# archibate/ptina

Measured on AMD Instinct MI355X. Metric: Msamples/sec (pixels x spp / s), 512x512x32spp cornell-monkey (978 tri), higher is better.
Workload: dtype f32; 1 GPU; s978: 978-tri synthetic cornell + bumpy sphere, 512x512, 32 spp, unidirectional MIS path tracer, depth<=5; step = 32 x render() + get_image() (resolve + D2H), exams/benchmark.py:29-36; spp=32, mode=fast, parallelism=single GPU

## Files before the change

### ptina_amd/csrc/lds_layout.h

```cpp
#pragma once

#if defined(__HIPCC__)
#define MPT_LDS_FN __host__ __device__ static inline
#else
#define MPT_LDS_FN static inline
#endif

#ifndef MPT_LDS_NODE_STRIDE
#define MPT_LDS_NODE_STRIDE 72
#endif
#ifndef MPT_LDS4_NODE_STRIDE
#define MPT_LDS4_NODE_STRIDE 112
#endif
#define MPT_LDS_MAT_VEC4 6

enum {
    MPT_LDS_BUDGET = 160 * 1024,
    MPT_LDS_LANES = 1024,
    MPT_LDS_LEVEL_BYTES = MPT_LDS_LANES * 2
};

typedef struct { int nnode4, ntri4, nmat4, nmtl4; } MptLdsRegions;

MPT_LDS_FN MptLdsRegions mpt_lds_regions(int n, int default_mtl) {
    MptLdsRegions r;
    r.nnode4 = ((n - 1) * MPT_LDS_NODE_STRIDE + 15) >> 4;
    r.ntri4 = n * 3;
    r.nmat4 = (default_mtl + 1) * MPT_LDS_MAT_VEC4;
    r.nmtl4 = (n + 15) >> 4;
    return r;
}

MPT_LDS_FN MptLdsRegions mpt_lds4_regions(int n, int nwide, int lds_nmats) {
    MptLdsRegions r;
    r.nnode4 = nwide * (MPT_LDS4_NODE_STRIDE / 16);
    r.ntri4 = (n + 1) * 3;
    r.nmat4 = (lds_nmats + 1) * MPT_LDS_MAT_VEC4;
    r.nmtl4 = (n + 15) >> 4;
    return r;
}

MPT_LDS_FN int mpt_lds_scene_vec4(MptLdsRegions r) { return r.nnode4 + r.ntri4 + r.nmat4 + r.nmtl4; }

MPT_LDS_FN int mpt_lds_launch_bytes(MptLdsRegions r, int stack_levels) {
    return mpt_lds_scene_vec4(r) * 16 + stack_levels * MPT_LDS_LEVEL_BYTES;
}

MPT_LDS_FN int mpt_lds_stack_levels(int fast_depth) { return fast_depth + 1; }

static inline int mpt_lds_fit_bytes(int n, int max_materials, int fast_depth) {
    if (n < 2) return 0;
    if (n >= 32768) return 0;
    if ((n - 1) * (MPT_LDS_NODE_STRIDE / 8) >= 32768) return 0;
    if (max_materials >= 256) return 0;
    if (fast_depth < 0 || fast_depth >= MPT_LDS_BUDGET / MPT_LDS_LEVEL_BYTES) return 0;
    const int bytes = mpt_lds_launch_bytes(mpt_lds_regions(n, max_materials), mpt_lds_stack_levels(fast_depth));
    return bytes <= MPT_LDS_BUDGET ? bytes : 0;
}

static inline int mpt_lds4_fit_bytes(int n, int nwide, int wide_stack, int lds_nmats) {
    if (n < 2 || nwide <= 0 || wide_stack <= 0) return 0;
    if (n >= 4095) return 0;
    if (nwide > 65535 / MPT_LDS4_NODE_STRIDE) return 0;
    if (lds_nmats < 0 || lds_nmats >= 255) return 0;
    if (wide_stack > MPT_LDS_BUDGET / MPT_LDS_LEVEL_BYTES) return 0;
    const int bytes = mpt_lds_launch_bytes(mpt_lds4_regions(n, nwide, lds_nmats), wide_stack);
    return bytes <= MPT_LDS_BUDGET ? bytes : 0;
}

enum { MPT_KERNEL_GATHER = 0, MPT_KERNEL_LDS = 1, MPT_KERNEL_WIDE = 2, MPT_KERNEL_LDS4 = 5 };

typedef struct {
    int fast;
    int use_lds;
    int lds_wide;
    int use_wide;
    int nfaces;
    int wide_nodes;
    int wide_stack;
    int have_wnode;
    int max_mtlid;
    int max_materials;
    int fast_depth;
} MptKernelFacts;

typedef struct { int kernel, lds_bytes; } MptKernelChoice;

static inline MptKernelChoice mpt_choose_kernel(const MptKernelFacts *f) {
    MptKernelChoice ch = { MPT_KERNEL_GATHER, 0 };
    if (!f->fast) return ch;
    if (f->use_lds) {
        if (f->lds_wide && f->use_wide && f->have_wnode)
            ch.lds_bytes = mpt_lds4_fit_bytes(f->nfaces, f->wide_nodes, f->wide_stack, f->max_mtlid + 1);
        if (ch.lds_bytes) { ch.kernel = MPT_KERNEL_LDS4; return ch; }
        ch.lds_bytes = mpt_lds_fit_bytes(f->nfaces, f->max_materials, f->fast_depth);
        if (ch.lds_bytes) { ch.kernel = MPT_KERNEL_LDS; return ch; }
    }
    if (f->use_wide && f->wide_nodes > 0) ch.kernel = MPT_KERNEL_WIDE;
    return ch;
}
```

### ptina_amd/csrc/miptina.cpp

```cpp

#include "miptina_ctx.h"
#include <chrono>

static int g_hwq = 0;
static bool g_hwq_late = false;
__attribute__((constructor)) static void mpt_want_hw_queues() {
    if (!getenv("GPU_MAX_HW_QUEUES")) {
        setenv("GPU_MAX_HW_QUEUES", "12", 0);
        const char *pre = getenv("LD_PRELOAD");
        if ((pre && strstr(pre, "rocprof")) || getenv("ROCP_TOOL_LIBRARIES")) {
            g_hwq_late = true;
            fprintf(stderr, "libmiptina: GPU_MAX_HW_QUEUES=12 requested after a preloaded profiler tool may have initialised HIP: "
                            "streams may fold onto the default 4 hardware queues (results unchanged; export the variable "
                            "before starting the profiler)\n");
        }
    }
    const char *v = getenv("GPU_MAX_HW_QUEUES");
    g_hwq = v ? atoi(v) : 0;
}

static thread_local std::string g_err;

int fail(const char *fmt, ...) {
    char buf[1024];
// ... 205 lines not shown

static bool is_locked_range(const void *p, size_t bytes) {
    std::lock_guard<std::mutex> lk(g_host_mu);
    auto it = g_host_bufs.upper_bound((uintptr_t)p);
    if (it == g_host_bufs.begin()) return false;
    --it;
    return (uintptr_t)p + bytes <= it->first + it->second;
}

static int read_back(mpt_ctx *c, void *out, const void *dev, size_t bytes) {
    if (is_locked_range(out, bytes)) {
        HIP_TRY(hipMemcpyAsync(out, dev, bytes, hipMemcpyDeviceToHost, c->stream));
        HIP_TRY(hipStreamSynchronize(c->stream));
        return 0;
    }
    if (bytes > c->h_stage_bytes) {
        if (c->h_stage) hipHostFree(c->h_stage);
        c->h_stage = nullptr; c->h_stage_bytes = 0;
        HIP_TRY(hipHostMalloc(&c->h_stage, bytes, hipHostMallocDefault));
        c->h_stage_bytes = bytes;
    }
    HIP_TRY(hipMemcpyAsync(c->h_stage, dev, bytes, hipMemcpyDeviceToHost, c->stream));
    HIP_TRY(hipStreamSynchronize(c->stream));
    memcpy(out, c->h_stage, bytes);
    return 0;
}

static int scene_feat_now(const mpt_ctx *c);

extern "C" int mpt_set_option(mpt_ctx *c, const char *key, int value) {
    if (use(c)) return 1;
    std::string k = key ? key : "";
    if (k == "mode") {
        if (value != MPT_MODE_FAST && value != MPT_MODE_STRICT) return fail("mode must be 0 (fast) or 1 (strict)");
        c->mode = value;
    } else if (k == "batch") {
        if (value < 1 || value > MPT_MAX_BATCH) return fail("batch must be in 1..%d", MPT_MAX_BATCH);
        c->batch = value;
    } else if (k == "chunk") {
        if (value < 0) return fail("chunk must be >= 0");
        c->chunk = value;
    } else if (k == "count") {
        c->count = value ? 1 : 0;
    } else if (k == "lds") {
        c->use_lds = value ? 1 : 0;
    } else if (k == "lds_wide") {
        if (value != 0 && value != 1) return fail("lds_wide must be 0 or 1");
        c->lds_wide = value;
    } else if (k == "zero_copy") {
        c->zero_copy = value ? 1 : 0;
    } else if (k == "shade_spec") {
        if (value != 0 && value != 1) return fail("shade_spec must be 0 (always the generic SHADE) or 1 (the plain one for plain scenes)");
        c->shade_spec = value;
    } else if (k == "skip_dark") {
        if (value < -1 || value > 1) return fail("skip_dark must be -1 (auto), 0 or 1");
        c->skip_dark = value;
    } else if (k == "spin_us") {
        if (value < 0) return fail("spin_us must be >= 0");
        c->spin_us = value;
    } else if (k == "finalise") {
        if (value < 0 || value > 2) return fail("finalise must be 0 (combine pass), 1 (tail finalisation) or 2 (the same without the early image: A/B)");
        c->finalise = value;
    } else if (k == "launch_seq") {
        if (value < 0) return fail("launch_seq must be >= 0");
        if (mpt_flush(c)) return 1;
        c->launch_seq = (unsigned)value;
        c->tag_epoch = 0xffffffffu;
    } else if (k == "timeline") {
        c->timeline = value ? 1 : 0;
    } else if (k == "pipe_depth") {
        if (value != 0 && (value < 2 || value > MPT_MAX_PIPE)) return fail("pipe_depth must be 0 (auto) or 2..%d", MPT_MAX_PIPE);
        c->pipe_depth = value;
    } else if (k == "grid_div") {
        if (value < 0 || value > 8) return fail("grid_div must be 0 (auto) or 1..8");
        c->grid_div = value;
    } else if (k == "lds_block") {
        if (value != 0 && value != 256 && value != 512 && value != 768 && value != 1024)
            return fail("lds_block must be 0 (auto), 256, 512, 768 or 1024");
        c->lds_block = value;
    } else if (k == "reserve_cus") {
        if (value < 0 || value >= c->num_cus) return fail("reserve_cus must be in 0..%d", c->num_cus - 1);
        c->reserve_cus = value;
    } else if (k == "wide") {
        c->use_wide = value ? 1 : 0;
    } else if (k == "sah_exact_max") {
        if (value < 2) return fail("sah_exact_max must be >= 2");
        c->sah_exact_max = value; c->tree_valid = false;
    } else if (k == "sah_build") {
        if (value < -1 || value > 1) return fail("sah_build must be -1 (auto), 0 (host) or 1 (device)");
        if (value != c->sah_build) { c->sah_build = value; c->tree_valid = false; }
    } else if (k == "wide_build") {
        if ((value ? 1 : 0) != c->wide_build) { c->wide_build = value ? 1 : 0; c->tree_valid = false; }
    } else if (k == "wide_quant") {
        c->use_quant = value ? 1 : 0;
    } else if (k == "tree") {
        if (value != 0 && value != 1) return fail("tree must be 0 (LBVH) or 1 (SAH)");
        if (value != c->tree_kind) { c->tree_kind = value; c->tree_valid = false; }
    } else if (k == "tile_w_shift" || k == "tile_h_shift") {
        if (value < 0 || value > 3) return fail("%s must be in 0..3", k.c_str());
        (k == "tile_w_shift" ? c->tile_w_shift : c->tile_h_shift) = value;
    } else if (k == "gpu_build") {
        if ((value ? 1 : 0) != c->gpu_build) { c->gpu_build = value ? 1 : 0; c->tree_valid = false; }
    } else if (k == "sah_inject_fail") {
        c->sah_inject_fail = value != 0; c->tree_valid = false;
    } else if (k == "build_phases") {
        c->build_phases = value ? 1 : 0;
    } else if (k == "lane_hist") {
        c->lane_hist = value ? 1 : 0;
    } else if (k == "sah_max") {
        c->sah_max = value; c->tree_valid = false;
    } else {
        return fail("unknown option '%s'", k.c_str());
    }
    return 0;
}

extern "C" int mpt_get_option(mpt_ctx *c, const char *key, int *value) {
    if (!c || !value) return fail("null argument");
    std::string k = key ? key : "";
    if (k == "mode") *value = c->mode;
    else if (k == "batch") *value = c->batch;
    else if (k == "chunk") *value = c->chunk;
    else if (k == "count") *value = c->count;
    else if (k == "tree_depth") *value = c->tree_depth;
    else if (k == "fast_depth") *value = c->fast_depth;
    else if (k == "tree") *value = c->tree_kind;
    else if (k == "gpu_build") *value = c->gpu_build;
    else if (k == "pending") *value = c->pending;
    else if (k == "lds") *value = c->use_lds;
    else if (k == "lds_wide") *value = c->lds_wide;
    else if (k == "lds_block") *value = c->lds_block;
    else if (k == "zero_copy") *value = c->zero_copy;
    else if (k == "spin_us") *value = c->spin_us;
    else if (k == "finalise") *value = c->finalise;
    else if (k == "last_finalised") *value = c->last_finalised;
    else if (k == "launch_seq") *value = (int)(c->launch_seq & 0x7fffffffu);
    else if (k == "tag_wraps") *value = (int)c->tag_wraps;
    else if (k == "skip_dark") *value = c->skip_dark;
    else if (k == "shade_spec") *value = c->shade_spec;
    else if (k == "scene_feat") *value = scene_feat_now(c);
    else if (k == "shade_inst") *value = c->last_shade_feat;
    else if (k == "pipe_depth") *value = c->pipe_depth;
    else if (k == "grid_div") *value = c->grid_div;
    else if (k == "cur_depth") *value = c->cur_depth;
    else if (k == "cur_div") *value = c->cur_div;
    else if (k == "last_div") *value = c->last_div;
    else if (k == "last_kernel") *value = c->last_kernel;
    else if (k == "num_cus") *value = c->num_cus;
    else if (k == "reserve_cus") *value = c->reserve_cus;
    else if (k == "wide") *value = c->use_wide;
    else if (k == "wide_quant") *value = c->use_quant;
    else if (k == "wide_build") *value = c->wide_build;
    else if (k == "sah_build") *value = c->sah_build;
    else if (k == "sah_fallback") *value = c->sah_fallback;
    else if (k == "build_phases") *value = c->build_phases;
    else if (k == "lane_hist") *value = c->lane_hist;
    else if (k == "sah_levels") *value = c->sah_stats.levels;
    else if (k == "sah_kelems") *value = (int)(c->sah_stats.elems / 1000);
    else if (k == "sah_chunks") *value = (int)c->sah_stats.chunks;
    else if (k == "sah_segments") *value = (int)c->sah_stats.segments;
    else if (k == "sah_part_kwords") *value = (int)(c->sah_stats.part_words / 1000);
    else if (k == "sah_tasks_small") *value = c->sah_stats.tasks_small;
    else if (k == "sah_tasks_big") *value = c->sah_stats.tasks_big;
    else if (k == "sah_t_sort_k") *value = c->sah_stats.t_sort_k;
    else if (k == "sah_t_loop_k") *value = c->sah_stats.t_loop_k;
    else if (k == "sah_t_max_k") *value = c->sah_stats.t_max_k;
    else if (k == "sah_task_levels") *value = c->sah_stats.task_levels;
    else if (k == "sah_task_levels_max") *value = c->sah_stats.task_levels_max;
    else if (k.rfind("build_phase_us_", 0) == 0 && k.size() == 16 && k[15] >= '0' && k[15] <= '5') *value = (int)(c->build_phase_us[k[15] - '0'] + 0.5);
    else if (k == "wide_nodes") *value = c->wide_nodes;
    else if (k == "wide_stack") *value = c->wide_stack;
    else if (k == "wide_ratio_permille") *value = (int)(c->wide_ratio * 1000.f + 0.5f);
    else if (k == "wide_depth") *value = c->wide_depth;
    else if (k == "nranks") *value = c->nranks;
    else if (k == "rank") *value = c->rank;
    else if (k == "device") *value = c->device;
    else if (k == "clock_khz") *value = c->clock_khz;
    else if (k == "hw_queues") *value = g_hwq_late ? -g_hwq : g_hwq;
    else return fail("unknown option '%s'", k.c_str());
    return 0;
}

extern "C" int mpt_set_size(mpt_ctx *c, int nx, int ny) {
    if (use(c)) return 1;
    if (nx <= 0 || ny <= 0) return fail("film size must be positive, got %dx%d", nx, ny);
    size_t npix = (size_t)nx * ny;
    if (npix > (size_t)c->caps.max_filmsize)
        return fail("film %dx%d exceeds max_filmsize=%d (init_things(max_filmsize=...))", nx, ny, c->caps.max_filmsize);
    if (npix > c->film_cap) {
        HIP_TRY(hipStreamSynchronize(c->stream));
        for (int p = 0; p < 3; p++) { hipFree(c->film[p]); c->film[p] = nullptr; }
        hipFree(c->resolved); c->resolved = nullptr;
// ... 519 lines not shown
    switch (kc.kernel) {
    case MPT_KERNEL_LDS4: HIP_TRY(mpt_launch_render_lds4(&p, launch_cus, lds_block, (size_t)kc.lds_bytes, c->count, shade_feat, s.rs)); break;
    case MPT_KERNEL_LDS: HIP_TRY(mpt_launch_render_lds(&p, launch_cus, lds_block, (size_t)kc.lds_bytes, c->count, s.rs)); break;
    case MPT_KERNEL_WIDE: HIP_TRY(mpt_launch_render_wide(&p, wide_blocks, c->count, c->use_quant, s.rs)); break;
    default:
        if (!s.fast) HIP_TRY(mpt_launch_render_strict(&p, p.ntiles, stack, c->count, s.rs));
        else HIP_TRY(mpt_launch_render_fast(&p, launch_cus, stack, c->count, s.rs));
    }
    c->last_shade_feat = shade_feat;
    c->last_kernel = kc.kernel;
    HIP_TRY(hipEventRecord(e1, s.rs));
    c->render_timer.record({ e0, e1 }, c->event_pool);
    return 0;
}

static int behind_launch(mpt_ctx *c, const MptRenderParams &p, const BatchSlot &s, int B, bool fin) {
    const int k = s.k;
    HIP_TRY(hipEventRecord(c->ev_render[k], s.rs));
    HIP_TRY(hipStreamWaitEvent(c->stream, c->ev_render[k], 0));
    if (!fin)
        HIP_TRY(mpt_launch_combine(c->film[0], c->partial2[k], c->ny, c->x0, c->x1, p.stripe_w, p.stripe_pitch,
                                   p.partial_stride / std::max(c->ny, 1), B, c->stream));
    HIP_TRY(hipEventRecord(c->ev_free[k], c->stream));
    const int k2 = c->flip % c->cur_depth;
    if (k2 != k) {
        HIP_TRY(hipStreamWaitEvent(s.ss, c->ev_render[k2], 0));
        HIP_TRY(mpt_launch_sobol_update(c->sX, c->sX_spec, c->sV, c->sP2[k2], c->sdim, c->srows, c->stime, B, B, 1, s.ss));
        HIP_TRY(hipMemsetAsync(c->d_work2[k2], 0, MPT_QUEUE_WORDS * sizeof(unsigned int), s.ss));
        HIP_TRY(hipEventRecord(c->ev_sobol2[k2], s.ss));
        c->spec_valid = true; c->spec_slot = k2; c->spec_B = B; c->spec_time = c->stime;
    }
    return 0;
}

extern "C" int mpt_flush(mpt_ctx *c) {
    if (!c) return fail("null context");
    if (c->mlt_pending && mlt_flush(c)) return 1;
    if (c->pending == 0) return 0;
    HIP_TRY(hipSetDevice(c->device));
    const int B = c->pending;
    c->pending = 0;
    MptRenderParams p;
    if (fill_params(c, p, B)) return 1;
    const bool fast = c->mode == MPT_MODE_FAST;
    if (fast && ring_policy(c, B)) return 1;
    BatchSlot s;
    s.fast = fast;
    s.k = fast ? (c->flip++ % c->cur_depth) : 0;
    s.rs = fast ? c->rstream[s.k] : c->stream;
    s.ss = fast ? c->aux : c->stream;
    bool use_spec = false;
    if (batch_points(c, p, s, B, &use_spec)) return 1;
    if (p.ntiles == 0) return 0;
    const MptKernelChoice kc = choose_kernel(c);
    p.lds_nmats = c->max_mtlid + 1;
    const int ccols = work_items(c, p, B, fast);
    if (fast && slab_and_queue_heads(c, p, s, B, ccols, use_spec)) return 1;
    bool ring_idle = false;
    int launch_cus = 0, wide_blocks = 0, lds_block = 0;
    if (launch_share(c, fast, &ring_idle, &launch_cus)) return 1;
    if (size_launch_buffers(c, p, s.k, kc.kernel, launch_cus, &wide_blocks, &lds_block)) return 1;
    const bool fin = fast && c->finalise && ring_idle && p.nitems > 0;
    if (setup_finalisation(c, p, s, fin)) return 1;
    if (launch_render(c, p, s, kc, launch_cus, lds_block, wide_blocks)) return 1;
    return fast ? behind_launch(c, p, s, B, fin) : 0;
}

extern "C" int mpt_render(mpt_ctx *c, int nframes) {
    if (!c) return fail("null context");
    if (nframes < 0) return fail("nframes must be >= 0");
    if (check_ready(c)) return 1;
    if (c->mlt_pending && mlt_flush(c)) return 1;
    while (nframes > 0) {
        int room = c->batch - c->pending;
        int take = std::min(room, nframes);
        c->pending += take;
        nframes -= take;
        if (c->pending >= c->batch && mpt_flush(c)) return 1;
    }
    return 0;
}

extern "C" int mpt_render_preview(mpt_ctx *c, int nframes) {
    if (use(c)) return 1;
    while (nframes > 0) {
        int B = std::min(nframes, MPT_MAX_BATCH);
        MptRenderParams p;
        if (fill_params(c, p, B)) return 1;
        if (sobol_advance(c, B, B)) return 1;
        p.chunk = B; p.nchunks = 1;
        const int stack = gather_stack_levels(c);
        if (p.ntiles) {
            if (c->mode == MPT_MODE_STRICT) HIP_TRY(mpt_launch_preview_strict(&p, p.ntiles, stack, c->stream));
            else HIP_TRY(mpt_launch_preview_fast(&p, p.ntiles, stack, c->stream));
        }
        nframes -= B;
    }
    return 0;
}

enum { MPT_MLT_SLAB_RECORDS = 1 << 24 };

static int mlt_check(mpt_ctx *c) {
    if (c->mlt_n <= 0) return fail("Metropolis engine not reset: call mpt_mlt_reset first");
    return 0;
}

// ... 440 lines not shown
```

### ptina_amd/csrc/miptina_ctx.h

```cpp
#pragma once

#include "../../include/miptina.h"
#include "mpt_types.h"
#include "shade_feat.h"
#include <hip/hip_runtime_api.h>
#include <rccl/rccl.h>
#include <dlfcn.h>
#include <algorithm>
#include <cmath>
#include <cstdarg>
#include <cstdio>
#include <chrono>
#include <cstring>
#include <initializer_list>
#include <map>
#include <mutex>
#include <string>
#include <vector>

MPT_KERNEL_API hipError_t mpt_launch_render_fast(const MptRenderParams *, int grid, int stack, int count, hipStream_t);
MPT_KERNEL_API hipError_t mpt_launch_render_strict(const MptRenderParams *, int grid, int stack, int count, hipStream_t);
MPT_KERNEL_API hipError_t mpt_launch_derive_materials(MptMaterial *mats, int count, hipStream_t);
MPT_KERNEL_API hipError_t mpt_launch_derive_tfast(const MptVec4 *tgeo, MptVec4 *tfast, int n, hipStream_t);
MPT_KERNEL_API hipError_t mpt_wide_blocks(int grid, int count, int quant, int *blocks);
// ... 53 lines not shown
#define MPT_INTERNAL __attribute__((visibility("hidden")))
MPT_INTERNAL int fail(const char *fmt, ...);

#define HIP_TRY(expr)                                                                     \
    do {                                                                                  \
        hipError_t e_ = (expr);                                                           \
        if (e_ != hipSuccess) return fail("%s failed: %s", #expr, hipGetErrorString(e_)); \
    } while (0)

struct MPT_INTERNAL MptLaunchTimer {
    const int per_launch;
    std::vector<hipEvent_t> events;
    explicit MptLaunchTimer(int n) : per_launch(n) {}

    void record(std::initializer_list<hipEvent_t> launch, std::vector<hipEvent_t> &pool) {
        for (hipEvent_t e : launch) events.push_back(e);
        if (events.size() > (size_t)per_launch * 4096) trim(pool);
    }
    void trim(std::vector<hipEvent_t> &pool) {
        const size_t half = (size_t)per_launch * 2048;
        for (size_t q = 0; q < half; q++) pool.push_back(events[q]);
        events.erase(events.begin(), events.begin() + half);
    }
    int drain(double *seg_ms, int *launches, std::vector<hipEvent_t> &pool) {
        for (size_t q = 0; q + per_launch <= events.size(); q += per_launch)
            for (int g = 0; g + 1 < per_launch; g++) {
                float t = 0;
                HIP_TRY(hipEventElapsedTime(&t, events[q + g], events[q + g + 1]));
                seg_ms[g] += t;
            }
        if (launches) *launches = (int)(events.size() / per_launch);
        for (hipEvent_t e : events) pool.push_back(e);
        events.clear();
        return 0;
    }
};

enum { MPT_MAX_PIPE = 6 };

struct mpt_ctx {
    int device = 0;
    hipStream_t stream = nullptr;
    mpt_caps caps{};

    int mode = MPT_MODE_FAST, batch = 32, chunk = 0, count = 0, use_lds = 1, lds_block = 0, zero_copy = 1;
    int lds_wide = 1;
    int skip_dark = -1;
    int max_mtlid = -1;
    int num_cus = 256;
    int clock_khz = 0;
    int tile_w_shift = 3, tile_h_shift = 3;
    int last_div = 1;
    int last_kernel = 0;
    int shade_spec = 1;
    int last_shade_feat = -1;

    int nx = 0, ny = 0, x0 = 0, x1 = 0;
    int stripe_w = 0, stripe_idx = 0, stripe_mod = 1;
    MptVec4 *film[3] = { nullptr, nullptr, nullptr };
    size_t film_cap = 0;
    MptVec4 *resolved = nullptr;
    float *exported = nullptr;

    int nfaces = 0;
    std::vector<float> verts;
    double scene_cen[3] = { 0, 0, 0 }, scene_rad = 0;
    std::vector<int32_t> mtlids;
    bool tree_valid = false;
    int tree_depth = 0;
    int fast_depth = 0;
    int tree_kind = 1;
    int gpu_build = 1;
    int sah_max = 1 << 22;
    bool host_tree_valid = false;
    float *d_verts = nullptr; int *d_mtlids = nullptr; size_t d_model_cap = 0;
    float *d_cen = nullptr; int *d_bounds = nullptr; int *d_depth = nullptr;
    unsigned long long *d_keys_in = nullptr, *d_keys_out = nullptr;
    void *d_sort_tmp = nullptr; size_t d_sort_bytes = 0;
    int *d_child = nullptr, *d_parent = nullptr, *d_leaf = nullptr, *d_mc = nullptr;
    float *d_bmin = nullptr, *d_bmax = nullptr;
    unsigned *d_arrive = nullptr;
    size_t d_build_cap = 0;
    std::vector<int32_t> h_child, h_leaf, h_mc;
    std::vector<float> h_bmin, h_bmax;
    MptVec4 *snode = nullptr, *fnode = nullptr, *tgeo = nullptr, *tshade = nullptr;
    MptVec4 *tfast = nullptr; size_t tfast_cap = 0;
    MptVec4 *qnode = nullptr; size_t qnode_cap = 0;
    int use_quant = 1;
    MptVec4 *wnode = nullptr; size_t wnode_cap = 0;
    int wide_nodes = 0, wide_depth = 0;
    int wide_stack = 0;
    float wide_ratio = 1.f;
    int sah_exact_max = 8192;
    int sah_inject_fail = 0;
    int *h_sahmeta = nullptr, *d_sahmeta = nullptr;
    MptSahStats sah_stats{};
    bool d_model_stale = true;
    int lane_hist = 0;
    int build_phases = 0;
    double build_phase_us[6] = { 0, 0, 0, 0, 0, 0 };
    int sah_fallback = 0;
    int sah_build = -1;
    void *sah_ws = nullptr; size_t sah_ws_bytes = 0;
    int wide_build = 1;
    int *wb_bin_of = nullptr, *wb_ncount = nullptr, *wb_offset = nullptr; void *wb_scan = nullptr; size_t wb_scan_bytes = 0;
    double *wb_area = nullptr; size_t wb_cap = 0;
// ... 108 lines not shown
```

### ptina_amd/csrc/mpt_types.h

```cpp
#pragma once

#include <stdint.h>

#define MPT_BLOCK 256
#define MPT_TILE 16
#define MPT_MAX_BATCH 64
#ifndef MPT_QUEUE_STRIDE
#define MPT_QUEUE_STRIDE 32
#endif
#define MPT_QUEUE_WORDS (10 * MPT_QUEUE_STRIDE)
#define MPT_TIMELINE_WORDS 8
#define MPT_MAX_LIGHTS 64
#define MPT_MAX_DEVICES 64

struct MptVec4 { float x, y, z, w; };

#define MPT_KERNEL_API extern "C" __attribute__((visibility("hidden")))

struct MptMaterial {
    float p[16];
    int32_t tex[12];
    int32_t any_tex;
    int32_t pad[3];
    float d[8];
};

struct MptLight {
    MptVec4 color_size;
    MptVec4 pos_type;
    MptVec4 ax0, ax1, ax2;
};

struct MptPiece { long long src, dst, count; };

struct MptSahStats {
    int levels;
    long long elems;
    long long chunks, segments;
    long long part_words;
    int tasks_small, tasks_big;
    int t_sort_k, t_loop_k, t_max_k;
    int task_levels, task_levels_max;
};

struct MptSahBuffers {
    const float *verts; const int *leaf; int n;
    MptVec4 *prim[2];
    int *seg[2]; size_t seg_cap;
    int *dec;
    int *ch_seg, *ch_left; size_t chunk_cap;
    int *part; size_t part_words;
    int *segbins; size_t segbin_words;
    int *tasks; size_t task_cap;
    int *meta;
    MptSahStats *stats;
    volatile int *mail_host; int *mail_dev;
    MptVec4 *fnode;
};

struct MptImage { int32_t nx, ny, base, pad; };

#include "lds_layout.h"

enum { MPT_TAG_COMBINE = 1, MPT_TAG_FIRST = 2, MPT_TAG_PERIOD = 65534 };
enum { MPT_HIST_BASE = 32, MPT_HIST_WORDS = 3 * 65 + 3 * 6 * 2 + 24, MPT_COUNTER_WORDS = MPT_HIST_BASE + MPT_HIST_WORDS };

struct MptRenderParams {
    int32_t nx, ny, x0, x1;
    int32_t nframes, chunk, nchunks, n;
    int32_t sobol_dim, nlights, world_tex, tiles_x;
    int32_t tiles_y, ntiles;
    float sobol_inv_dim;
    int32_t nitems, tile_w_shift, tile_h_shift;
    int32_t nwide;
    int32_t stripe_w, stripe_pitch;
    int32_t partial_stride;
    int32_t lds_nmats;
    int32_t skip_dark;
    int32_t default_mtl;
    float world_fac[4];
    float v2w[16];
    const MptVec4 *snode;
    const MptVec4 *fnode;
    const MptVec4 *wnode;
    const MptVec4 *qnode;
    const MptVec4 *tgeo;
    const MptVec4 *tshade;
    const MptVec4 *tfast;
    const MptMaterial *mats;
    const MptLight *lights;
    const MptImage *images;
    const MptVec4 *texels;
    const float *P;
    MptVec4 *film0;
    MptVec4 *film1;
    MptVec4 *film2;
    MptVec4 *partial;
    unsigned long long *counters;
    unsigned int *work_counter;
    int *stack_spill;
    unsigned int *watchdog;
    unsigned int *fin_counter;
    MptVec4 *image_out;
    uint32_t slab_tag;
    int32_t lane_hist;
    float t_scale, t_unscale;
    int32_t pad3;
    unsigned long long *timeline;
};

struct MptMltArgs {
    float *X;
    float *L;
    int32_t *bit;
    uint32_t *keys;
    MptVec4 *vals;
    int32_t nchains, t0, K;
    uint32_t seed;
    float lsp, sigma;
};
```

### ptina_amd/csrc/render_kernel.hip

```cpp

#include "pt_device.h"
#include "film_ops.h"
#include <atomic>

#if MPT_STRICT
#define MPT_SUFFIX(x) x##_strict
#else
#define MPT_SUFFIX(x) x##_fast
#endif

#include "path_common.h"

template <bool COUNT>
DEV void flush_counters(const MptRenderParams &p, const Cnt &c) {
    if (!COUNT) return;
    unsigned v[20] = { c.samples, c.rays, c.n_box, c.n_tri, c.n_shade, c.n_draws, c.bounces, c.n_node,
                       c.it_node, c.it_leaf, c.it_shade, c.it_new,
                       c.pl_local, c.pl_batches, c.pl_batch_lanes, c.pl_prim, c.pl_tidle, c.pl_sidle, c.pl_trips, c.pl_taken };
#pragma unroll
    for (int k = 0; k < 20; k++) {
        unsigned x = v[k];
#pragma unroll
        for (int off = 32; off > 0; off >>= 1) x += __shfl_xor(x, off);
        if ((threadIdx.x & 63) == 0 && x) atomicAdd(p.counters + k, (unsigned long long)x);
// ... 366 lines not shown
        rec = shade_rec_load<SCENE::LDS_MATS>(p, hslot);
        lane_draws<6, SCENE::LDS_MATS>(p, L, u);
    }
    MPT_SEG(pl_trips)
    LightHit lit = lights_hit<FEAT>(p, ro, rd);
    if (lit.hit && (!was_hit || lit.dis < hdepth)) {
        float mis = power_heuristic(L.last_brdf_pdf, lit.pdf);
        L.result = L.result + L.throughput * (lit.color * mis);
    }
    hitpos = ro; sdir = v3s(0.0f); sdis = 0.0f;
    MPT_SEG(pl_local)
    if (!was_hit) {
        L.result = L.result + L.throughput * world_at<FEAT>(p, rd);
        L.depth = 5;
        return SH_END;
    }
    L.navoid = SCENE::ODD_IDS ? L.hidx : ~L.hidx;
    Hit hit; hit.hit = 1; hit.depth = hdepth; hit.index = hslot; hit.u = L.hu; hit.v = L.hv;
    V3 normal; Disney mat;
    get_geometries_rec<FEAT>(p, sc, rec, hit, ro, rd, &hitpos, &normal, mat);
    if (COUNT) { cnt.n_shade++; cnt.n_draws += 6; }
    float sign = -dot(rd, normal);
    if (sign < 0.0f) normal = -normal;
    MPT_SEG(pl_batches)

    LightSample li = lights_sample<FEAT>(p, hitpos, v3(u[0], u[1], u[2]));
    bool want_shadow = any_gt0(li.color);
    MPT_SEG(pl_batch_lanes)
    L.direct = v3s(0.0f);
    if (want_shadow) {
        V3 brdf_clr = disney_brdf<FEAT>(mat, normal, sign, -rd, li.dir);
        float brdf_pdf = vavg(brdf_clr);
        float mis = power_heuristic(li.pdf, brdf_pdf);
        V3 direct_li = li.color * mis * brdf_clr * dot_or_zero(normal, li.dir);
        L.direct = L.throughput * direct_li;
    }
    MPT_SEG(pl_prim)
    BsdfSample brdf = disney_bounce<FEAT>(mat, normal, sign, -rd, v3(u[3], u[4], u[5]));
    L.throughput = L.throughput * brdf.color;
    L.prd = brdf.outdir;
    L.last_brdf_pdf = brdf.pdf;
    MPT_SEG(pl_tidle)
    if (want_shadow && p.n >= 2 && (p.skip_dark == 0 || any_ne0(L.direct))) {
        sdir = li.dir; sdis = li.dis;
        return SH_SHADOW;
    }
    if (want_shadow && p.n < 2) { L.result = L.result + L.direct; if (COUNT) cnt.rays++; }
    return SH_BOUNCE;
}

struct PrimaryPool {
    V3 ro, rd;
    int rng_i, rng_k;
};
DEV void pool_prepare(const MptRenderParams &p, PrimaryPool &pp, bool inside, int i, int j, int frame) {
    pp.ro = v3s(0.0f); pp.rd = v3s(0.0f); pp.rng_i = 0; pp.rng_k = -1;
    if (inside) {
        LaneState T;
        T.frame = frame;
        T.rng_i = wanghash2(i, j);
        T.rng_k = reduce_mod_dim(T.rng_i, p.sobol_dim, p.sobol_inv_dim);
        float jit[2];
        lane_draws<2>(p, T, jit);
        float x = m_div((float)i + jit[0], (float)p.nx) * 2.0f - 1.0f;
        float y = m_div((float)j + jit[1], (float)p.ny) * 2.0f - 1.0f;
        camera_generate(p, x, y, &pp.ro, &pp.rd);
        pp.rng_i = T.rng_i; pp.rng_k = T.rng_k;
    }
}
DEV float lane_from(float v, int byte_lane) { return __int_as_float(__builtin_amdgcn_ds_bpermute(byte_lane, __float_as_int(v))); }
DEV int lane_from(int v, int byte_lane) { return __builtin_amdgcn_ds_bpermute(byte_lane, v); }

#ifndef MPT_PREF_NODE
#define MPT_PREF_NODE 1
#define MPT_PREF_LEAF 1
#endif
#ifndef MPT_LEAVE_A
#define MPT_LEAVE_A 2
#define MPT_LEAVE_B 1
#endif
#if MPT_X_STAMPS
#define MPT_STAMP_BEGIN unsigned long long stamp_t0 = 0; if (COUNT) { __builtin_amdgcn_sched_barrier(0); stamp_t0 = __builtin_amdgcn_s_memtime(); __builtin_amdgcn_sched_barrier(0); }
#define MPT_STAMP_END(acc) if (COUNT) { __builtin_amdgcn_sched_barrier(0); acc += __builtin_amdgcn_s_memtime() - stamp_t0; __builtin_amdgcn_sched_barrier(0); }
#else
#define MPT_STAMP_BEGIN
#define MPT_STAMP_END(acc)
#endif
DEV void lane_hist_add(const MptRenderParams &p, int stage, bool part, int depth, int shadow) {
    unsigned long long *h = p.counters + MPT_HIST_BASE;
    const bool l0 = (threadIdx.x & 63) == 0;
    const int n = (int)__builtin_popcountll(__ballot(part));
    if (l0) atomicAdd(h + stage * 65 + n, 1ull);
    for (int d = 0; d < 6; d++)
        for (int k = 0; k < 2; k++) {
            const int c = (int)__builtin_popcountll(__ballot(part && min(depth, 5) == d && (shadow != 0) == (k != 0)));
            if (l0 && c) atomicAdd(h + 3 * 65 + (stage * 6 + d) * 2 + k, (unsigned long long)c);
        }
}
DEV void node_id_hist_add(const MptRenderParams &p, bool part, int id) {
    unsigned long long *h = p.counters + MPT_HIST_BASE + 3 * 65 + 3 * 6 * 2;
    const int b = id <= 0 ? 0 : 32 - __builtin_clz((unsigned)id);
    for (int k = 0; k < 24; k++) {
        const int c = (int)__builtin_popcountll(__ballot(part && b == k));
        if ((threadIdx.x & 63) == 0 && c) atomicAdd(h + k, (unsigned long long)c);
    }
}
DEV int wave_count(bool pred) { return (int)__builtin_popcountll(__ballot(pred)); }
DEV int wave_count32(bool pred) {
    unsigned long long m = __ballot(pred);
    int n;
    asm("s_bcnt1_i32_b64 %0, %1" : "=s"(n) : "s"(m) : "scc");
    return n;
}

struct WorkQueue {
    unsigned int *ctr;
    int nitems, q0, qoff;
    DEV int pull() {
        const int lane = threadIdx.x & 63;
        while (qoff < 8) {
            int q = (q0 + qoff) & 7;
            int lo = (int)(((long long)nitems * q) >> 3), hi = (int)(((long long)nitems * (q + 1)) >> 3);
            int k = 0;
            if (lane == 0) k = (int)atomicAdd(ctr + q * MPT_QUEUE_STRIDE, 1u);
            k = __builtin_amdgcn_readfirstlane(k);
            if (lo + k < hi) return lo + k;
            qoff++;
        }
        return -1;
    }
};

template <bool COUNT, int FEAT, class SCENE, class STACK>
DEV void trace_stream(const MptRenderParams &p, const SCENE &sc, STACK stk, WorkQueue wq, Cnt &cnt,
                      unsigned long long *tl = nullptr) {
    const int tws = p.tile_w_shift, ths = p.tile_h_shift, tps = tws + ths;
    const int t8y = (p.ny + (1 << ths) - 1) >> ths;
    int S = 0, next = 0;
    int ti = 0, tj = 0, f0 = 0, tx_cur = 0;
    int ndead = 0;
    int deferred = 0;
    bool more = true;
    PrimaryPool pool;
    pool.ro = v3s(0.0f); pool.rd = v3s(0.0f); pool.rng_i = 0; pool.rng_k = -1;
    int pool_base = -64;
#if MPT_X_TIMELINE2
    int tl_items = 0, tl_passes = 0;
    unsigned long long tl_lastpull = 0;
#endif
#if MPT_X_STAMPS
    unsigned long long acc_node = 0, acc_leaf = 0, acc_sdone = 0, acc_shade = 0, acc_new = 0;
    const unsigned long long stamp_start = __builtin_amdgcn_s_memtime();
#endif
    LaneState L;
    L.st = ST_NEW;
    L.sp = 0; L.curr = 0; L.shadow = 0;
    L.result = v3s(0.0f); L.throughput = v3s(0.0f); L.prd = v3s(0.0f); L.direct = v3s(0.0f);
    L.to = v3s(0.0f); L.td = v3s(0.0f); L.inv = v3s(0.0f); L.oinv = v3s(0.0f);
    L.offx = 0; L.offy = 0; L.offz = 0;
    L.tbest = 0.0f; L.hidx = -1; L.hu = 0.0f; L.hv = 0.0f; L.last_brdf_pdf = 0.0f;
    L.navoid = 0; L.depth = 0; L.rng_i = 0; L.rng_k = 0; L.pix = 0; L.frame = 0;
    for (unsigned guard = 0;; guard++) {
        if (guard > (1u << 26)) {
            if ((threadIdx.x & 63) == 0) __hip_atomic_store(p.watchdog, 1u, __ATOMIC_RELAXED, __HIP_MEMORY_SCOPE_SYSTEM);
            break;
        }
        for (;;) {
            const int cn = wave_count32(L.st == ST_NODE);
            const int cl = wave_count32(L.st == ST_LEAF);
            const int trav = cn + cl;
            if (trav == 0) break;
            if (trav * MPT_LEAVE_A < (64 - ndead - trav - deferred) * MPT_LEAVE_B) break;
            MPT_STAMP_BEGIN
#if MPT_X_PAIRS
            const unsigned long long mn = __ballot(L.st == ST_NODE), ml = __ballot(L.st == ST_LEAF);
            if (COUNT && (threadIdx.x & 63) == 0) {
                if (cn * MPT_PREF_NODE >= cl * MPT_PREF_LEAF) { cnt.pl_local += (unsigned)__builtin_popcount((unsigned)mn | (unsigned)(mn >> 32)); cnt.pl_prim += (unsigned)__builtin_popcountll(mn); cnt.pl_trips++; }
                else { cnt.pl_batches += (unsigned)__builtin_popcount((unsigned)ml | (unsigned)(ml >> 32)); cnt.pl_tidle += (unsigned)__builtin_popcountll(ml); cnt.pl_taken++; }
            }
#endif
            if (cn * MPT_PREF_NODE >= cl * MPT_PREF_LEAF) {
                if (COUNT && (threadIdx.x & 63) == 0) cnt.it_node++;
                if (COUNT && p.lane_hist) lane_hist_add(p, 0, L.st == ST_NODE, L.depth, L.shadow);
                if constexpr (!STACK::ODD_IDS) { if (COUNT && p.lane_hist) node_id_hist_add(p, L.st == ST_NODE, L.curr); }
                if (L.st == ST_NODE) {
                    if constexpr (SCENE::WIDE) stage_node4<COUNT>(sc, stk, L, cnt);
                    else stage_node<COUNT>(sc, stk, L, cnt);
                }
#pragma unroll
                for (int rep = 0; rep < SCENE::NODE_REP; rep++) {
                    if (__ballot(L.st == ST_NODE) == 0ull) break;
                    if (COUNT && (threadIdx.x & 63) == 0) cnt.it_node++;
                    if (COUNT && p.lane_hist) lane_hist_add(p, 0, L.st == ST_NODE, L.depth, L.shadow);
                    if constexpr (!STACK::ODD_IDS) { if (COUNT && p.lane_hist) node_id_hist_add(p, L.st == ST_NODE, L.curr); }
                    if (L.st == ST_NODE) {
                        if constexpr (SCENE::WIDE) stage_node4<COUNT>(sc, stk, L, cnt);
                        else stage_node<COUNT>(sc, stk, L, cnt);
// ... 46 lines not shown
            if (L.st == ST_DONE && L.shadow) {
                if (L.hidx < 0) L.result = L.result + L.direct;
                L.st = ST_BOUNCE;
            }
            if (L.st == ST_BOUNCE && !path_continues(L)) lane_store_sample(p, L);
            MPT_STAMP_END(acc_sdone)
        }
        MPT_STAMP_BEGIN
        unsigned long long m_new = __ballot(L.st == ST_NEW);
        if (m_new != 0ull) {
            if (next >= S && more) {
#if MPT_X_STAMPS == 3
                const unsigned long long tp0 = __builtin_amdgcn_s_memtime();
#endif
                int item = wq.pull();
#if MPT_X_STAMPS == 3
                if (COUNT && (threadIdx.x & 63) == 0) cnt.pl_local += (unsigned)((__builtin_amdgcn_s_memtime() - tp0) >> 4);
#endif
                if (item < 0) {
                    more = false;
                    if (tl && (threadIdx.x & 63) == 0) {
                        tl[2] = wall_clock64();
#if MPT_X_TIMELINE2
                        tl[4] = tl_lastpull; tl[5] = (unsigned long long)tl_items;
                        tl[6] = (unsigned long long)(64 - (int)__builtin_popcountll(m_new));
#endif
                    }
                } else {
#if MPT_X_TIMELINE2
                    tl_items++; tl_lastpull = wall_clock64();
#endif
                    int tile = item / p.nchunks, chunk = item - tile * p.nchunks;
                    int tx = tile / t8y, ty = tile - tx * t8y;
                    int tps_x = p.stripe_w >> tws, st = tx / tps_x;
                    ti = p.x0 + st * p.stripe_pitch + ((tx - st * tps_x) << tws); tj = ty << ths; tx_cur = tx;
                    f0 = chunk * p.chunk;
                    S = (min(f0 + p.chunk, p.nframes) - f0) << tps;
                    next = 0; pool_base = -64;
                }
            }
            if (next < S) {
                if (COUNT && (threadIdx.x & 63) == 0) cnt.it_new++;
                const int lane = threadIdx.x & 63;
                if (next >= pool_base + 64) {
                    pool_base = next;
                    const int smp = pool_base + lane;
                    const int q = smp & ((1 << tps) - 1);
                    const int i = ti + (q >> ths), j = tj + (q & ((1 << ths) - 1));
#if MPT_X_STAMPS == 3
                    __builtin_amdgcn_sched_barrier(0);
                    const unsigned long long tq0 = __builtin_amdgcn_s_memtime();
#endif
                    pool_prepare(p, pool, smp < S && i < p.x1 && j < p.ny, i, j, f0 + (smp >> tps));
#if MPT_X_STAMPS == 3
                    {
                        float sink = pool.rd.x + pool.ro.x;
                        asm volatile("" :: "v"(sink));
                        __builtin_amdgcn_sched_barrier(0);
                        if (COUNT && (threadIdx.x & 63) == 0) cnt.pl_batches += (unsigned)((__builtin_amdgcn_s_memtime() - tq0) >> 4);
                    }
#endif
                }
                const int rank = __builtin_amdgcn_mbcnt_hi((unsigned)(m_new >> 32), __builtin_amdgcn_mbcnt_lo((unsigned)m_new, 0u));
                const int smp = next + rank;
                const int pool_end = min(S, pool_base + 64);
                const int src = ((smp - pool_base) & 63) << 2;
                V3 ro = v3(lane_from(pool.ro.x, src), lane_from(pool.ro.y, src), lane_from(pool.ro.z, src));
                V3 rd = v3(lane_from(pool.rd.x, src), lane_from(pool.rd.y, src), lane_from(pool.rd.z, src));
                const int rng_i = lane_from(pool.rng_i, src), rng_k = lane_from(pool.rng_k, src);
                if (L.st == ST_NEW && smp < pool_end && rng_k >= 0) {
                    const int q = smp & ((1 << tps) - 1);
                    L.frame = f0 + (smp >> tps);
                    L.pix = ((tx_cur << tws) + (q >> ths)) * p.ny + (tj + (q & ((1 << ths) - 1)));
                    L.rng_i = rng_i; L.rng_k = rng_k; L.prd = rd;
                    L.navoid = 0; L.depth = 0;
                    L.result = v3s(0.0f); L.throughput = v3s(1.0f); L.last_brdf_pdf = 0.0f;
                    if (COUNT) { cnt.samples++; cnt.n_draws += 2; }
                    L.to = ro;
                    L.st = ST_BOUNCE;
                    if (!path_continues(L)) lane_store_sample(p, L);
                }
                next = min(next + (int)__builtin_popcountll(m_new), pool_end);
            } else if (!more) {
                if (L.st == ST_NEW) L.st = ST_DEAD;
                ndead += (int)__builtin_popcountll(m_new);
            }
        }
        MPT_STAMP_END(acc_new)
        {
            MPT_STAMP_BEGIN
            if (L.st == ST_BOUNCE || L.st == ST_SHADOW) lane_begin_ray<COUNT>(p, L, stk, cnt);
            MPT_STAMP_END(acc_sdone)
        }
#if MPT_X_TIMELINE2
        if (!more) tl_passes++;
        if (ndead == 64 && tl && (threadIdx.x & 63) == 0) tl[7] = (unsigned long long)tl_passes;
#endif
        if (ndead == 64) break;
    }
#if MPT_X_STAMPS
    if (COUNT) {
        const bool l0 = (threadIdx.x & 63) == 0;
        const unsigned long long total = __builtin_amdgcn_s_memtime() - stamp_start;
        cnt.n_box = l0 ? (unsigned)(acc_node >> 8) : 0u; cnt.n_tri = l0 ? (unsigned)(acc_leaf >> 8) : 0u;
        cnt.n_draws = l0 ? (unsigned)(acc_sdone >> 8) : 0u; cnt.n_shade = l0 ? (unsigned)(acc_shade >> 8) : 0u;
        cnt.bounces = l0 ? (unsigned)(acc_new >> 8) : 0u; cnt.n_node = l0 ? (unsigned)(total >> 8) : 0u;
    }
#endif
}

DEV mpt_u4 slab_load_sc1(const MptVec4 *frame_base, unsigned frame_bytes, unsigned byte_off) {
    const __amdgpu_buffer_rsrc_t rsrc = __builtin_amdgcn_make_buffer_rsrc((void *)frame_base, (short)0, (int)frame_bytes, 0x00020000);
#ifndef MPT_FIN_AUX
#define MPT_FIN_AUX 16
#endif
    return __builtin_amdgcn_raw_buffer_load_b128(rsrc, (int)byte_off, 0, MPT_FIN_AUX);
}

#ifndef MPT_FIN_SLEEP
#define MPT_FIN_SLEEP 32
#endif
#ifndef MPT_FIN_GROUP_LDS
#define MPT_FIN_GROUP_LDS 8
#define MPT_FIN_GROUP_GATHER 6
#endif
struct FinArgs {
    MptVec4 *partial, *film0, *image_out;
    unsigned int *fin_counter, *watchdog;
    int tile_w_shift, tile_h_shift, ny, nitems, nchunks, nframes, partial_stride, stripe_w, stripe_pitch, x0, x1;
    unsigned slab_tag;
};
DEV int uniform_i(int v) { return __builtin_amdgcn_readfirstlane(v); }
template <class T> DEV T *uniform_p(T *ptr) {
// ... 402 lines not shown
```

Baseline: 3742 Msamples/s.

## Pretrace a pool's 64 camera rays together before handing them to lanes

When a wave refills its primary-ray pool in the LDS wide-BVH kernel for plain scenes, it now traces all 64 camera rays as one coherent batch. It uses spare LDS stack levels above the lanes' in-flight stacks. Each lane that then picks up a new sample gets the precomputed hit and goes straight to shading, skipping its own divergent primary traversal. The cost is extra LDS per block, which may lower occupancy, plus a synchronous batch trace that stalls in-flight lanes. Rays that overflow the reserved stack fall back to per-lane tracing.

Result: slower. 3576 Msamples/s (-4.4%).

```diff
diff --git a/ptina_amd/csrc/lds_layout.h b/ptina_amd/csrc/lds_layout.h
--- a/ptina_amd/csrc/lds_layout.h
+++ b/ptina_amd/csrc/lds_layout.h
@@ -68,6 +68,14 @@
     return bytes <= MPT_LDS_BUDGET ? bytes : 0;
 }
 
+static inline int mpt_lds4_pretrace_levels(int fit_bytes, int wide_stack, int cap) {
+    if (fit_bytes <= 0 || fit_bytes > MPT_LDS_BUDGET || wide_stack <= 0) return 0;
+    int extra = (MPT_LDS_BUDGET - fit_bytes) / MPT_LDS_LEVEL_BYTES;
+    if (extra > wide_stack) extra = wide_stack;
+    if (cap >= 0 && extra > cap) extra = cap;
+    return extra;
+}
+
 enum { MPT_KERNEL_GATHER = 0, MPT_KERNEL_LDS = 1, MPT_KERNEL_WIDE = 2, MPT_KERNEL_LDS4 = 5 };
 
 typedef struct {
diff --git a/ptina_amd/csrc/miptina.cpp b/ptina_amd/csrc/miptina.cpp
--- a/ptina_amd/csrc/miptina.cpp
+++ b/ptina_amd/csrc/miptina.cpp
@@ -281,6 +281,12 @@
     } else if (k == "shade_spec") {
         if (value != 0 && value != 1) return fail("shade_spec must be 0 (always the generic SHADE) or 1 (the plain one for plain scenes)");
         c->shade_spec = value;
+    } else if (k == "pretrace") {
+        if (value != 0 && value != 1) return fail("pretrace must be 0 (every lane traces its own camera ray) or 1 (a pool's 64 camera rays are traced together)");
+        c->pretrace = value;
+    } else if (k == "pretrace_levels") {
+        if (value < -1) return fail("pretrace_levels must be -1 (auto) or >= 0");
+        c->pretrace_levels = value;
     } else if (k == "skip_dark") {
         if (value < -1 || value > 1) return fail("skip_dark must be -1 (auto), 0 or 1");
         c->skip_dark = value;
@@ -367,6 +373,9 @@
     else if (k == "tag_wraps") *value = (int)c->tag_wraps;
     else if (k == "skip_dark") *value = c->skip_dark;
     else if (k == "shade_spec") *value = c->shade_spec;
+    else if (k == "pretrace") *value = c->pretrace;
+    else if (k == "pretrace_levels") *value = c->pretrace_levels;
+    else if (k == "pretrace_extra") *value = c->last_pretrace_extra;
     else if (k == "scene_feat") *value = scene_feat_now(c);
     else if (k == "shade_inst") *value = c->last_shade_feat;
     else if (k == "pipe_depth") *value = c->pipe_depth;
@@ -992,7 +1001,14 @@
     bool use_spec = false;
     if (batch_points(c, p, s, B, &use_spec)) return 1;
     if (p.ntiles == 0) return 0;
-    const MptKernelChoice kc = choose_kernel(c);
+    MptKernelChoice kc = choose_kernel(c);
+    c->last_pretrace_extra = 0;
+    if (kc.kernel == MPT_KERNEL_LDS4 && c->pretrace && shade_feat_instantiation(scene_feat_now(c), c->shade_spec) == MPT_FEAT_PLAIN) {
+        const int extra = mpt_lds4_pretrace_levels(kc.lds_bytes, c->wide_stack, c->pretrace_levels);
+        kc.lds_bytes = mpt_lds_launch_bytes(mpt_lds4_regions(c->nfaces, c->wide_nodes, c->max_mtlid + 1), c->wide_stack + extra);
+        p.pre_levels = c->wide_stack + extra;
+        c->last_pretrace_extra = extra;
+    }
     p.lds_nmats = c->max_mtlid + 1;
     const int ccols = work_items(c, p, B, fast);
     if (fast && slab_and_queue_heads(c, p, s, B, ccols, use_spec)) return 1;
diff --git a/ptina_amd/csrc/miptina_ctx.h b/ptina_amd/csrc/miptina_ctx.h
--- a/ptina_amd/csrc/miptina_ctx.h
+++ b/ptina_amd/csrc/miptina_ctx.h
@@ -129,6 +129,9 @@
     int tile_w_shift = 3, tile_h_shift = 3;
     int last_div = 1;
     int last_kernel = 0;
+    int pretrace = 1;
+    int pretrace_levels = -1;
+    int last_pretrace_extra = 0;
     int shade_spec = 1;
     int last_shade_feat = -1;
 
diff --git a/ptina_amd/csrc/mpt_types.h b/ptina_amd/csrc/mpt_types.h
--- a/ptina_amd/csrc/mpt_types.h
+++ b/ptina_amd/csrc/mpt_types.h
@@ -63,7 +63,8 @@
 #include "lds_layout.h"
 
 enum { MPT_TAG_COMBINE = 1, MPT_TAG_FIRST = 2, MPT_TAG_PERIOD = 65534 };
-enum { MPT_HIST_BASE = 32, MPT_HIST_WORDS = 3 * 65 + 3 * 6 * 2 + 24, MPT_COUNTER_WORDS = MPT_HIST_BASE + MPT_HIST_WORDS };
+enum { MPT_HIST_BASE = 32, MPT_HIST_BATCH = 3 * 65 + 3 * 6 * 2 + 24, MPT_HIST_WORDS = MPT_HIST_BATCH + 2 * 65 + 2,
+       MPT_COUNTER_WORDS = MPT_HIST_BASE + MPT_HIST_WORDS };
 
 struct MptRenderParams {
     int32_t nx, ny, x0, x1;
@@ -105,7 +106,7 @@
     uint32_t slab_tag;
     int32_t lane_hist;
     float t_scale, t_unscale;
-    int32_t pad3;
+    int32_t pre_levels;
     unsigned long long *timeline;
 };
 
diff --git a/ptina_amd/csrc/render_kernel.hip b/ptina_amd/csrc/render_kernel.hip
--- a/ptina_amd/csrc/render_kernel.hip
+++ b/ptina_amd/csrc/render_kernel.hip
@@ -442,7 +442,10 @@
 struct PrimaryPool {
     V3 ro, rd;
     int rng_i, rng_k;
+    float tbest, hu, hv;
+    int hidx;
 };
+enum { POOL_UNTRACED = -2 };
 DEV void pool_prepare(const MptRenderParams &p, PrimaryPool &pp, bool inside, int i, int j, int frame) {
     pp.ro = v3s(0.0f); pp.rd = v3s(0.0f); pp.rng_i = 0; pp.rng_k = -1;
     if (inside) {
@@ -487,6 +490,10 @@
             if (l0 && c) atomicAdd(h + 3 * 65 + (stage * 6 + d) * 2 + k, (unsigned long long)c);
         }
 }
+DEV void lane_hist_add_batch(const MptRenderParams &p, int stage, bool part) {
+    const int n = (int)__builtin_popcountll(__ballot(part));
+    if ((threadIdx.x & 63) == 0) atomicAdd(p.counters + MPT_HIST_BASE + MPT_HIST_BATCH + stage * 65 + n, 1ull);
+}
 DEV void node_id_hist_add(const MptRenderParams &p, bool part, int id) {
     unsigned long long *h = p.counters + MPT_HIST_BASE + 3 * 65 + 3 * 6 * 2;
     const int b = id <= 0 ? 0 : 32 - __builtin_clz((unsigned)id);
@@ -501,6 +508,64 @@
     int n;
     asm("s_bcnt1_i32_b64 %0, %1" : "=s"(n) : "s"(m) : "scc");
     return n;
+}
+
+DEV V3 camera_dir_normalized(V3 a) {
+    const float s = __builtin_fmaf(a.z, a.z, __builtin_fmaf(a.y, a.y, a.x * a.x));
+    return a * m_rnorm(s);
+}
+template <int FEAT, class SCENE, class STACK>
+constexpr bool pretrace_built() { return STACK::SP_ADDR && STACK::ODD_IDS && SCENE::WIDE && FEAT == MPT_FEAT_PLAIN; }
+
+template <bool COUNT, class SCENE, class STACK>
+DEV void pool_trace(const MptRenderParams &p, const SCENE &sc, STACK &stk, PrimaryPool &pp, int sp0, int sp_lim, Cnt &cnt) {
+    LaneState B;
+    Cnt bc = {};
+    B.st = ST_DEAD; B.navoid = 0; B.depth = 1; B.shadow = 0;
+    B.tbest = 0.0f; B.hidx = -1; B.hu = 0.0f; B.hv = 0.0f; B.curr = 0; B.sp = sp0;
+    B.to = pp.ro; B.td = pp.rd; B.inv = pp.rd; B.oinv = pp.rd;
+    if (pp.rng_k >= 0 && any_ne0(pp.rd) && sp0 <= sp_lim) {
+        lane_start_ray<false>(B, stk, pp.ro, camera_dir_normalized(pp.rd), MPT_INF, false, bc);
+        STACK::st(sp0, STACK::SENTINEL);
+        B.sp = sp0;
+    }
+    for (;;) {
+        const int cn = wave_count32(B.st == ST_NODE);
+        const int cl = wave_count32(B.st == ST_LEAF);
+        if (cn + cl == 0) break;
+        if (cn * MPT_PREF_NODE >= cl * MPT_PREF_LEAF) {
+            if (COUNT && (threadIdx.x & 63) == 0) cnt.it_node++;
+            if (B.st == ST_NODE && B.sp > sp_lim) B.st = ST_DEAD;
+            if (COUNT && p.lane_hist) lane_hist_add_batch(p, 0, B.st == ST_NODE);
+            if (B.st == ST_NODE) stage_node4<COUNT>(sc, stk, B, bc);
+#pragma unroll
+            for (int rep = 0; rep < SCENE::NODE_REP; rep++) {
+                if (B.st == ST_NODE && B.sp > sp_lim) B.st = ST_DEAD;
+                if (__ballot(B.st == ST_NODE) == 0ull) break;
+                if (COUNT && (threadIdx.x & 63) == 0) cnt.it_node++;
+                if (COUNT && p.lane_hist) lane_hist_add_batch(p, 0, B.st == ST_NODE);
+                if (B.st == ST_NODE) stage_node4<COUNT>(sc, stk, B, bc);
+            }
+        } else {
+            if (COUNT && (threadIdx.x & 63) == 0) cnt.it_leaf++;
+            if (COUNT && p.lane_hist) lane_hist_add_batch(p, 1, B.st == ST_LEAF);
+            if (B.st == ST_LEAF) stage_leaf<COUNT>(sc, stk, B, bc);
+#pragma unroll
+            for (int rep = 0; rep < SCENE::LEAF_REP; rep++) {
+                if (__ballot(B.st == ST_LEAF) == 0ull) break;
+                if (COUNT && (threadIdx.x & 63) == 0) cnt.it_leaf++;
+                if (COUNT && p.lane_hist) lane_hist_add_batch(p, 1, B.st == ST_LEAF);
+                if (B.st == ST_LEAF) stage_leaf<COUNT>(sc, stk, B, bc);
+            }
+        }
+    }
+    const bool traced = B.st == ST_DONE;
+    pp.hidx = traced ? B.hidx : (int)POOL_UNTRACED;
+    pp.tbest = B.tbest; pp.hu = B.hu; pp.hv = B.hv;
+    if (COUNT && traced) {
+        cnt.rays++; cnt.bounces++;
+        cnt.n_node += bc.n_node; cnt.n_box += bc.n_box; cnt.n_tri += bc.n_tri;
+    }
 }
 
 struct WorkQueue {
@@ -533,6 +598,8 @@
     bool more = true;
     PrimaryPool pool;
     pool.ro = v3s(0.0f); pool.rd = v3s(0.0f); pool.rng_i = 0; pool.rng_k = -1;
+    constexpr bool PRETRACE = pretrace_built<FEAT, SCENE, STACK>();
+    if constexpr (PRETRACE) { pool.tbest = 0.0f; pool.hu = 0.0f; pool.hv = 0.0f; pool.hidx = POOL_UNTRACED; }
     int pool_base = -64;
 #if MPT_X_TIMELINE2
     int tl_items = 0, tl_passes = 0;
@@ -685,6 +752,13 @@
                     const unsigned long long tq0 = __builtin_amdgcn_s_memtime();
 #endif
                     pool_prepare(p, pool, smp < S && i < p.x1 && j < p.ny, i, j, f0 + (smp >> tps));
+                    if constexpr (PRETRACE) {
+                        pool.hidx = POOL_UNTRACED;
+                        if (p.pre_levels > 0) {
+                            const bool flying = L.st == ST_NODE || L.st == ST_LEAF;
+                            pool_trace<COUNT>(p, sc, stk, pool, flying ? L.sp + STACK::SP_STEP : stk.sp_at(0), stk.sp_at(p.pre_levels - 4), cnt);
+                        }
+                    }
 #if MPT_X_STAMPS == 3
                     {
                         float sink = pool.rd.x + pool.ro.x;
@@ -701,6 +775,14 @@
                 V3 ro = v3(lane_from(pool.ro.x, src), lane_from(pool.ro.y, src), lane_from(pool.ro.z, src));
                 V3 rd = v3(lane_from(pool.rd.x, src), lane_from(pool.rd.y, src), lane_from(pool.rd.z, src));
                 const int rng_i = lane_from(pool.rng_i, src), rng_k = lane_from(pool.rng_k, src);
+                int pre_hidx = POOL_UNTRACED;
+                float pre_tbest = 0.0f, pre_hu = 0.0f, pre_hv = 0.0f;
+                if constexpr (PRETRACE) {
+                    if (p.pre_levels > 0) {
+                        pre_hidx = lane_from(pool.hidx, src); pre_tbest = lane_from(pool.tbest, src);
+                        pre_hu = lane_from(pool.hu, src); pre_hv = lane_from(pool.hv, src);
+                    }
+                }
                 if (L.st == ST_NEW && smp < pool_end && rng_k >= 0) {
                     const int q = smp & ((1 << tps) - 1);
                     L.frame = f0 + (smp >> tps);
@@ -712,6 +794,16 @@
                     L.to = ro;
                     L.st = ST_BOUNCE;
                     if (!path_continues(L)) lane_store_sample(p, L);
+                    if constexpr (PRETRACE) {
+                        if (COUNT && p.lane_hist && p.pre_levels > 0 && L.st == ST_BOUNCE)
+                            atomicAdd(p.counters + MPT_HIST_BASE + MPT_HIST_BATCH + 2 * 65 + (pre_hidx != POOL_UNTRACED ? 0 : 1), 1ull);
+                        if (L.st == ST_BOUNCE && pre_hidx != POOL_UNTRACED) {
+                            L.prd = camera_dir_normalized(rd);
+                            L.depth = 1; L.shadow = 0;
+                            L.tbest = pre_tbest; L.hidx = pre_hidx; L.hu = pre_hu; L.hv = pre_hv;
+                            L.st = ST_DONE;
+                        }
+                    }
                 }
                 next = min(next + (int)__builtin_popcountll(m_new), pool_end);
             } else if (!more) {
```
